# jeffersonfparil/poolgen

Measured on AMD Instinct MI355X. Metric: loci/sec ols_iter_with_kinship, 200 pools x 10M loci, higher is better.
Workload: dtype f64

## Files before the change

### poolgen_amd/csrc/pg_kinship.hip

```cpp
#include "pg_common.h"
#include <cstdlib>
#include <cstring>
#include <utility>

namespace {

#ifndef KIN_WAVES_DEF
#define KIN_WAVES_DEF 16
#endif
constexpr int KIN_WAVES = KIN_WAVES_DEF;
constexpr int KIN_THREADS = 64 * KIN_WAVES;
#ifndef KIN_RING_D
#define KIN_RING_D 3
#endif
constexpr int KIN_FUSE_MAXK = 2;
constexpr int KIN_TPW = 96 / KIN_WAVES;
#ifndef KIN_KC_DEF
#define KIN_KC_DEF 16
#endif
constexpr int KIN_KC = KIN_KC_DEF;
constexpr int KIN_PPT = (KIN_KC * 128 + KIN_THREADS - 1) / KIN_THREADS;

typedef double double4_t __attribute__((ext_vector_type(4)));
typedef unsigned int uint4_t __attribute__((ext_vector_type(4)));
typedef unsigned int uint2_t __attribute__((ext_vector_type(2)));

template <int CTRL, int ROW_MASK>
__device__ __forceinline__ double dpp_add(double v) {
    const int lo = __builtin_amdgcn_update_dpp(0, __double2loint(v), CTRL, ROW_MASK, 0xf, true);
    const int hi = __builtin_amdgcn_update_dpp(0, __double2hiint(v), CTRL, ROW_MASK, 0xf, true);
    return v + __hiloint2double(hi, lo);
}
template <int N>
__device__ __forceinline__ double row_from_plus(double v) {
    static_assert(N >= 1 && N <= 15, "row rotation");
    constexpr int CTRL = 0x120 + (16 - N);
    const int lo = __builtin_amdgcn_update_dpp(0, __double2loint(v), CTRL, 0xf, 0xf, false);
    const int hi = __builtin_amdgcn_update_dpp(0, __double2hiint(v), CTRL, 0xf, 0xf, false);
    return __hiloint2double(hi, lo);
}
template <int... I, typename F>
__device__ __forceinline__ void static_for_impl(std::integer_sequence<int, I...>, F &&f) {
    (f(std::integral_constant<int, I>{}), ...);
}
template <int N, typename F>
__device__ __forceinline__ void static_for(F &&f) {
    static_for_impl(std::make_integer_sequence<int, N>{}, f);
}
constexpr int kin_tri_ti(int t, int T) { int ti = 0; while (ti < T && t >= T - ti) { t -= T - ti; ++ti; } return ti < T ? ti : 0; }
constexpr int kin_tri_tj(int t, int T) { int ti = 0; while (ti < T && t >= T - ti) { t -= T - ti; ++ti; } return ti < T ? ti + t : 0; }
constexpr int kin_slot_tile(int w, int u, int T) { return (w + KIN_WAVES_DEF * u) < T * (T + 1) / 2 ? (w + KIN_WAVES_DEF * u) : 0; }

constexpr int KIN13_T[16][6][2] = {
    {{0, 0}, {0, 1}, {0, 2}, {1, 1}, {1, 2}, {2, 2}},
    {{3, 3}, {3, 4}, {3, 5}, {4, 4}, {4, 5}, {5, 5}},
    {{6, 6}, {6, 7}, {6, 8}, {7, 7}, {7, 8}, {8, 8}},
    {{9, 9}, {9, 10}, {9, 11}, {10, 10}, {10, 11}, {11, 11}},
    {{0, 3}, {0, 4}, {0, 5}, {1, 3}, {1, 4}, {1, 5}},
    {{0, 6}, {0, 7}, {0, 8}, {1, 6}, {1, 7}, {1, 8}},
    {{0, 9}, {0, 10}, {0, 11}, {1, 9}, {1, 10}, {1, 11}},
    {{3, 6}, {3, 7}, {3, 8}, {4, 6}, {4, 7}, {4, 8}},
    {{3, 9}, {3, 10}, {3, 11}, {4, 9}, {4, 10}, {4, 11}},
    {{6, 9}, {6, 10}, {6, 11}, {7, 9}, {7, 10}, {7, 11}},
    {{2, 4}, {2, 11}, {2, 12}, {4, 12}, {11, 12}, {12, 12}},
    {{2, 5}, {2, 6}, {2, 7}, {5, 6}, {5, 7}, {-1, -1}},
    {{0, 12}, {2, 3}, {3, 12}, {6, 12}, {7, 12}, {-1, -1}},
    {{5, 9}, {5, 10}, {5, 12}, {9, 12}, {10, 12}, {-1, -1}},
    {{2, 8}, {2, 9}, {2, 10}, {8, 9}, {8, 10}, {-1, -1}},
    {{1, 12}, {5, 8}, {5, 11}, {8, 11}, {8, 12}, {-1, -1}},
};
constexpr int kin13_ntiles(int w) { int c = 0; for (int u = 0; u < 6; ++u) c += KIN13_T[w][u][0] >= 0; return c; }
constexpr int kin13_col(int w, int idx) {
    int seen[12] = {-1, -1, -1, -1, -1, -1, -1, -1, -1, -1, -1, -1}, ns = 0;
    for (int u = 0; u < 6; ++u)
        for (int h = 0; h < 2; ++h) {
            const int c = KIN13_T[w][u][h];
            if (c < 0) continue;
            bool dup = false;
            for (int i = 0; i < ns; ++i) dup = dup || seen[i] == c;
            if (!dup) seen[ns++] = c;
        }
    return idx < ns ? seen[idx] : -1;
}
constexpr int kin13_ncols(int w) { int c = 0; while (c < 12 && kin13_col(w, c) >= 0) ++c; return c; }
constexpr int kin13_slot(int w, int col) { int i = 0; while (kin13_col(w, i) != col) ++i; return i; }
constexpr int KIN13_MAXC = 6;
constexpr int kin13_ndiag(int w) { int c = 0; for (int u = 0; u < 6; ++u) c += (KIN13_T[w][u][0] >= 0 && KIN13_T[w][u][0] == KIN13_T[w][u][1]); return c; }
constexpr int kin13_diag_index(int w, int u) { int c = 0; for (int v = 0; v < u; ++v) c += (KIN13_T[w][v][0] >= 0 && KIN13_T[w][v][0] == KIN13_T[w][v][1]); return c; }

struct KinParams {
    const double *G;
    int64_t p;
    int64_t ld;
    int64_t loci_per_wg;
    double *slabs;
    int n, T, npad, Tb, nb;
    int split;
    int merged;
    const double *ytil;
    double *spec;
    int k;
    int xcd_spx, npairs, nslab;
    int skip_dead;
    int wq_n[6], wq_first[6];
    int64_t wq_len[6];
};

template <bool FUSE, bool SPEC13, int SMALL = 0, bool SKIP = false, bool ODDN = true>
__global__ __launch_bounds__(KIN_THREADS, 1) void k_kinship_syrk(KinParams P) {
    extern __shared__ __attribute__((aligned(16))) double lds[];
    const int tid = threadIdx.x;
    const int lane = tid & 63;
    const int wave = tid >> 6;
    const int fi = lane & 15;
    const int kq = lane >> 4;

    int bx = blockIdx.x, by = blockIdx.y;
    if (P.xcd_spx) {
        const int xcd = blockIdx.x & 7, s = blockIdx.x >> 3, main = P.xcd_spx * P.npairs;
        if (s < main) { bx = xcd * P.xcd_spx + s / P.npairs; by = s % P.npairs; }
        else { const int e = (s - main) * 8 + xcd; bx = 8 * P.xcd_spx + e / P.npairs; by = e % P.npairs; }
        if (bx >= P.nslab) return;
    }
    int64_t loci_per_wg = P.loci_per_wg;
    if (P.wq_n[0] > 0) {
        int q = 0;
        while (q + 1 < P.npairs && (int)blockIdx.x >= P.wq_first[q + 1]) ++q;
        by = q;
        bx = (int)blockIdx.x - P.wq_first[q];
        loci_per_wg = P.wq_len[q];
    }
    int bi = 0, bj = 0;
    {
        int q = by / P.split;
        const int first = P.merged ? 1 : 0;
        for (bi = 0; bi < P.nb; ++bi) {
            const int cnt = P.nb - bi - first;
            if (q < cnt) { bj = bi + first + q; break; }
            q -= cnt;
        }
    }
    const bool diag = (bi == bj);
    const int Ta = min(P.Tb, P.T - bi * P.Tb);
    const int Tbb = min(P.Tb, P.T - bj * P.Tb);
    const int colsA = Ta * 16;
    const int colsB = diag ? 0 : Tbb * 16;
    int ldsld = colsA + colsB;
    if ((ldsld & 31) != 16) ldsld += 16;
    const int a0 = bi * P.Tb * 16;
    const int b0 = bj * P.Tb * 16;
    const int wa = min(colsA, P.n - a0);
    const int wb = diag ? 0 : min(colsB, P.n - b0);
    const int npa = (wa + 1) >> 1, npb = (wb + 1) >> 1;
    const int npr = npa + npb;

    const int nrect = diag ? 0 : Ta * Tbb;
    const int NA = Ta * (Ta + 1) / 2, NB = Tbb * (Tbb + 1) / 2, part = P.nb - 1;
    const int rankA = bj - 1, rankB = bi;
    const int cntA = P.merged ? (NA > rankA ? (NA - rankA + part - 1) / part : 0) : 0;
    const int cntB = P.merged ? (NB > rankB ? (NB - rankB + part - 1) / part : 0) : 0;
    const int ntiles = diag ? NA : nrect + cntA + cntB;
    const int split_id = by % P.split;
    int acol[KIN_TPW], bcol[KIN_TPW], orow[KIN_TPW], ocol[KIN_TPW];
    bool live[KIN_TPW];
#pragma unroll
    for (int u = 0; u < KIN_TPW; ++u) {
        const int t = split_id + P.split * (wave + KIN_WAVES * u);
        int ti = 0, tj = 0;
        live[u] = t < ntiles;
        int kind = diag ? 1 : 0;
        if (t < ntiles) {
            int q = t, Td = Ta;
            if (!diag && t >= nrect) {
                const bool inA = t - nrect < cntA;
                kind = inA ? 1 : 2;
                q = inA ? rankA + part * (t - nrect) : rankB + part * (t - nrect - cntA);
                Td = inA ? Ta : Tbb;
            }
            if (kind) {
                for (ti = 0; ti < Td; ++ti) {
                    const int cnt = Td - ti;
                    if (q < cnt) { tj = ti + q; break; }
                    q -= cnt;
                }
            } else {
                ti = t / Tbb;
                tj = t - ti * Tbb;
            }
        }
        acol[u] = (kind == 2 ? colsA : 0) + 16 * ti;
        bcol[u] = (kind == 1 ? 0 : colsA) + 16 * tj;
        orow[u] = (kind == 2 ? b0 : a0) + 16 * ti;
        ocol[u] = (kind == 1 ? a0 : b0) + 16 * tj;
    }

    int st_loc[KIN_PPT], st_lcol[KIN_PPT];
    int st_gcol[KIN_PPT];
    bool st_on[KIN_PPT], st_two[KIN_PPT];
#pragma unroll
    for (int r = 0; r < KIN_PPT; ++r) {
        const int t = tid + r * KIN_THREADS;
        const int loc = t / npr;
        const int q = t - loc * npr;
        st_on[r] = loc < KIN_KC;
        st_loc[r] = loc;
        int gcol, lcol;
        bool two;
        if (q < npa) {
            gcol = a0 + 2 * q; lcol = 2 * q; two = (2 * q + 1) < wa;
        } else {
            const int q2 = q - npa;
            gcol = b0 + 2 * q2; lcol = colsA + 2 * q2; two = (2 * q2 + 1) < wb;
        }
        st_lcol[r] = lcol;
        st_two[r] = two;
        st_gcol[r] = st_on[r] ? gcol : a0;
        if (!st_on[r]) st_loc[r] = 0;
    }

    const int64_t l_begin = (int64_t)bx * loci_per_wg;
    const int64_t l_end = min(P.p, l_begin + loci_per_wg);
    const int nstages = (l_end > l_begin) ? (int)((l_end - l_begin + KIN_KC - 1) / KIN_KC) : 0;
    const int bufsz = KIN_KC * ldsld;

    for (int i = tid; i < 2 * bufsz; i += KIN_THREADS) lds[i] = 0.0;
    double *ylds = lds + 2 * bufsz;
    if (FUSE)
        for (int i = tid; i < P.k * 256; i += KIN_THREADS) ylds[i] = P.ytil[i];
    __syncthreads();

    const uint64_t slab_bytes64 = (uint64_t)(l_end > l_begin ? l_end - l_begin : 0) * P.ld * 8;
    const __amdgpu_buffer_rsrc_t rsrc = __builtin_amdgcn_make_buffer_rsrc(
        const_cast<double *>(P.G + l_begin * P.ld), 0, (int)(uint32_t)slab_bytes64, 0x00020000);
    uint4_t stage_reg[KIN_PPT];
    uint32_t st_voff[KIN_PPT];
#pragma unroll
    for (int r = 0; r < KIN_PPT; ++r)
        st_voff[r] = st_on[r] ? (uint32_t)(((int64_t)st_loc[r] * P.ld + st_gcol[r]) * 8) : 0xFFFFFFF0u;
    const uint32_t stage_stride = (uint32_t)(KIN_KC * P.ld * 8);
    auto stage_load = [&](int c) {
#pragma unroll
        for (int r = 0; r < KIN_PPT; ++r)
            stage_reg[r] = __builtin_amdgcn_raw_buffer_load_b128(
                rsrc, st_on[r] ? st_voff[r] + (uint32_t)c * stage_stride : 0xFFFFFFF0u, 0, 0);
    };
    auto stage_store = [&](int buf) {
#pragma unroll
        for (int r = 0; r < KIN_PPT; ++r) {
            if (st_on[r]) {
                uint4_t v = stage_reg[r];
                if (!st_two[r]) { v.z = 0u; v.w = 0u; }
                *reinterpret_cast<uint4_t *>(&lds[buf * bufsz + st_loc[r] * ldsld + st_lcol[r]]) = v;
            }
        }
    };

    if (nstages > 0) {
        stage_load(0);
        stage_store(0);
    }
    __syncthreads();

    const int NV = 2 + P.k;
    double *scratch = ylds + KIN_FUSE_MAXK * 256 + wave * (4 * 64);
    double yreg[KIN_FUSE_MAXK][4];
#pragma unroll
    for (int t = 0; t < KIN_FUSE_MAXK; ++t)
#pragma unroll
        for (int j = 0; j < 4; ++j) yreg[t][j] = (FUSE && t < P.k) ? ylds[t * 256 + lane + 64 * j] : 0.0;
    auto spec_pass = [&](const double *buf, int64_t lbase) {
#pragma unroll
        for (int jl = 0; jl < KIN_KC / KIN_WAVES; ++jl) {
            const int loc = wave + KIN_WAVES * jl;
            const double *row = buf + loc * ldsld;
            const double shift = row[0];
            double s1 = 0.0, s2 = 0.0, sy[KIN_FUSE_MAXK], d[4];
#pragma unroll
            for (int t = 0; t < KIN_FUSE_MAXK; ++t) sy[t] = 0.0;
#pragma unroll
            for (int j = 0; j < 4; ++j) {
                const int pool = lane + 64 * j;
                if (SPEC13 && j < 3) d[j] = row[pool] - shift;
                else {
                    const double gv = row[pool < ldsld ? pool : ldsld - 1];
                    d[j] = (pool < P.n) ? gv - shift : 0.0;
                }
                s1 += d[j];
                s2 = fma(d[j], d[j], s2);
                sy[0] = fma(d[j], yreg[0][j], sy[0]);
            }
            const bool two = P.k > 1;
            if (two) {
#pragma unroll
                for (int j = 0; j < 4; ++j) sy[1] = fma(d[j], yreg[1][j], sy[1]);
            }
            scratch[lane] = s1;
            scratch[64 + lane] = s2;
            scratch[2 * 64 + lane] = sy[0];
            if (two) scratch[3 * 64 + lane] = sy[1];
            __builtin_amdgcn_wave_barrier();
            const int v = lane >> 4, r = lane & 15;
            const double *sc = scratch + v * 64 + r;
            double tot = (sc[0] + sc[16]) + (sc[32] + sc[48]);
            tot = dpp_add<0x111, 0xf>(tot);
            tot = dpp_add<0x112, 0xf>(tot);
            tot = dpp_add<0x114, 0xf>(tot);
            tot = dpp_add<0x118, 0xf>(tot);
            const int64_t l = lbase + loc;
            if (r == 15 && v < NV && l < l_end) P.spec[l * NV + v] = tot;
            __builtin_amdgcn_wave_barrier();
        }
    };

    auto run = [&](auto wc, auto tc) {
        constexpr int W = decltype(wc)::value;
        constexpr int TPW = decltype(tc)::value;
        constexpr int KS = KIN_KC / 4;
        constexpr int NQ = KS * TPW;
        constexpr int D = KIN_RING_D, R = KIN_RING_D + 1;
        static_assert(NQ % R == 0 && NQ > 2 * D, "ring indexing assumes the stage length is a multiple of the ring");
        double4_t acc[TPW];
#pragma unroll
        for (int u = 0; u < TPW; ++u) acc[u] = (double4_t){0.0, 0.0, 0.0, 0.0};
#ifndef KIN_SHARED_FRAGS
#define KIN_SHARED_FRAGS 1
#endif
        if constexpr (W >= 0 && KIN_SHARED_FRAGS) {
            constexpr int NC = kin13_ncols(W), NT = kin13_ntiles(W);
            static_assert(NC <= KIN13_MAXC && KS % 2 == 0, "fragment sets alternate with the k-step parity");
            constexpr int LD13 = 208, BUF13 = KIN_KC * LD13;
            auto ldv = [](const double *q) __attribute__((always_inline)) { return *(const volatile __attribute__((address_space(3))) double *)q; };
            double fr[2][KIN13_MAXC];
            const double *lb = lds + kq * LD13 + fi;
            constexpr bool has_strip = [] { bool h = false; for (int u = 0; u < 6; ++u) h = h || (KIN13_T[W][u][0] >= 0 && KIN13_T[W][u][0] < 12 && KIN13_T[W][u][1] == 12); return h; }();
            double bs[2][2];
            const double *lbs = lds + kq * LD13 + 192 + (lane & 3);
            constexpr int ND = (SMALL & 1) ? kin13_ndiag(W) : 0;
            double bd[2][ND > 0 ? ND : 1][2];
            const double *lbr1 = lds + kq * LD13 + ((fi + 4) & 15), *lbr2 = lds + kq * LD13 + ((fi + 8) & 15);
            auto load_set = [&](auto bc, auto sc, auto pc) __attribute__((always_inline)) {
                constexpr int s2 = decltype(sc)::value, par = decltype(pc)::value;
                constexpr int o = decltype(bc)::value * BUF13 + 4 * s2 * LD13;
                static_for<NC>([&](auto cc) __attribute__((always_inline)) {
                    constexpr int ci = decltype(cc)::value;
                    fr[par][ci] = ldv(lb + (o + 16 * kin13_col(W, ci)));
                });
                if constexpr ((SMALL & 2) != 0 && has_strip) {
                    bs[par][0] = ldv(lbs + o);
                    bs[par][1] = ldv(lbs + (o + 4));
                }
                if constexpr (ND > 0) {
                    static_for<NT>([&](auto uc) __attribute__((always_inline)) {
                        constexpr int u = decltype(uc)::value;
                        if constexpr (KIN13_T[W][u][0] == KIN13_T[W][u][1]) {
                            constexpr int di = kin13_diag_index(W, u);
                            bd[par][di][0] = ldv(lbr1 + (o + 16 * KIN13_T[W][u][0]));
                            bd[par][di][1] = ldv(lbr2 + (o + 16 * KIN13_T[W][u][0]));
                        }
                    });
                }
            };
            auto mfma_set = [&](auto pc) __attribute__((always_inline)) {
                constexpr int par = decltype(pc)::value;
                static_for<NT>([&](auto uc) __attribute__((always_inline)) {
                    constexpr int u = decltype(uc)::value;
                    constexpr int ti = KIN13_T[W][u][0], tj = KIN13_T[W][u][1];
                    const double fa = fr[par][kin13_slot(W, ti)];
                    if constexpr ((SMALL & 1) != 0 && ti == tj) {
                        acc[u][0] = __builtin_amdgcn_mfma_f64_4x4x4f64(fa, fa, acc[u][0], 0, 0, 0);
                        acc[u][1] = __builtin_amdgcn_mfma_f64_4x4x4f64(fa, bd[par][kin13_diag_index(W, u)][0], acc[u][1], 0, 0, 0);
                        acc[u][2] = __builtin_amdgcn_mfma_f64_4x4x4f64(fa, bd[par][kin13_diag_index(W, u)][1], acc[u][2], 0, 0, 0);
                    } else if constexpr ((SMALL & 2) != 0 && tj == 12 && ti != tj) {
                        acc[u][0] = __builtin_amdgcn_mfma_f64_4x4x4f64(fa, bs[par][0], acc[u][0], 0, 0, 0);
                        acc[u][1] = __builtin_amdgcn_mfma_f64_4x4x4f64(fa, bs[par][1], acc[u][1], 0, 0, 0);
                    } else {
                        acc[u] = __builtin_amdgcn_mfma_f64_16x16x4f64(fa, fr[par][kin13_slot(W, tj)], acc[u], 0, 0, 0);
                    }
                });
            };
            constexpr auto st_kind = [](int r) { const int t0 = W * 64 + r * KIN_THREADS; return t0 + 63 < KIN_KC * 97 ? 2 : (t0 >= KIN_KC * 104 ? 0 : 1); };
            uint4_t sreg[KIN_PPT];
            uint32_t voff[KIN_PPT];
            uint4_t *sdst[KIN_PPT];
#pragma unroll
            for (int r = 0; r < KIN_PPT; ++r) {
                sreg[r] = (uint4_t){0u, 0u, 0u, 0u};
                voff[r] = st_voff[r];
                sdst[r] = reinterpret_cast<uint4_t *>(&lds[st_loc[r] * LD13 + st_lcol[r]]);
            }
            auto st_load = [&]() __attribute__((always_inline)) {
                static_for<KIN_PPT>([&](auto rc) __attribute__((always_inline)) {
                    constexpr int r = decltype(rc)::value;
                    if constexpr (st_kind(r) == 2) {
                        voff[r] += stage_stride;
                        sreg[r] = __builtin_amdgcn_raw_buffer_load_b128(rsrc, voff[r], 0, 0);
                    } else if constexpr (st_kind(r) == 1) {
                        if (st_on[r]) {
                            voff[r] += stage_stride;
                            sreg[r] = __builtin_amdgcn_raw_buffer_load_b128(rsrc, voff[r], 0, 0);
                        }
                    }
                });
            };
            auto st_store = [&](auto bc) __attribute__((always_inline)) {
                constexpr int B = decltype(bc)::value;
                static_for<KIN_PPT>([&](auto rc) __attribute__((always_inline)) {
                    constexpr int r = decltype(rc)::value;
                    if constexpr (st_kind(r) != 0) {
                        uint4_t v = sreg[r];
                        if constexpr (ODDN) {
                            if (!st_two[r]) { v.z = 0u; v.w = 0u; }
                        }
                        if (st_kind(r) == 2 || st_on[r]) sdst[r][B * (BUF13 / 2)] = v;
                    }
                });
            };
            const double *srow = lds + lane, *srow3 = lds + (lane + 192 < P.n ? lane + 192 : 0);
            const bool sp_on = (lane & 15) == 15 && (lane >> 4) < NV;
            uint32_t sp_voff = (uint32_t)((W * NV + (lane >> 4)) * 8);
            const uint32_t sp_stride = (uint32_t)(KIN_KC * NV * 8);
            const __amdgpu_buffer_rsrc_t srsrc = __builtin_amdgcn_make_buffer_rsrc(
                FUSE ? P.spec + l_begin * NV : nullptr, 0, FUSE ? (int)(uint32_t)((uint64_t)(l_end > l_begin ? l_end - l_begin : 0) * NV * 8) : 0, 0x00020000);
            const double *sc13 = scratch + (lane >> 4) * 64 + (lane & 15);
            auto spec13 = [&](auto bc) __attribute__((always_inline)) {
                static_for<KIN_KC / KIN_WAVES>([&](auto jc) __attribute__((always_inline)) {
                    constexpr int jl = decltype(jc)::value;
                    constexpr int ro = decltype(bc)::value * BUF13 + (W + KIN_WAVES * jl) * LD13;
                    const double shift = ldv(lds + ro);
                    double s1 = 0.0, s2 = 0.0, sy[KIN_FUSE_MAXK], d[4];
#pragma unroll
                    for (int t = 0; t < KIN_FUSE_MAXK; ++t) sy[t] = 0.0;
#pragma unroll
                    for (int j = 0; j < 4; ++j) {
                        d[j] = (j < 3 ? ldv(srow + (ro + 64 * j)) : ldv(srow3 + ro)) - shift;
                        s1 += d[j];
                        s2 = fma(d[j], d[j], s2);
                        sy[0] = fma(d[j], yreg[0][j], sy[0]);
                    }
                    const bool two = P.k > 1;
                    if (two) {
#pragma unroll
                        for (int j = 0; j < 4; ++j) sy[1] = fma(d[j], yreg[1][j], sy[1]);
                    }
                    scratch[lane] = s1;
                    scratch[64 + lane] = s2;
                    scratch[2 * 64 + lane] = sy[0];
                    if (two) scratch[3 * 64 + lane] = sy[1];
                    __builtin_amdgcn_wave_barrier();
                    double tot = (sc13[0] + sc13[16]) + (sc13[32] + sc13[48]);
                    tot = dpp_add<0x111, 0xf>(tot);
                    tot = dpp_add<0x112, 0xf>(tot);
                    tot = dpp_add<0x114, 0xf>(tot);
                    tot = dpp_add<0x118, 0xf>(tot);
                    if (sp_on)
                        __builtin_amdgcn_raw_buffer_store_b64((uint2_t){(uint32_t)__double2loint(tot), (uint32_t)__double2hiint(tot)}, srsrc,
                                                              sp_voff + (uint32_t)(KIN_WAVES * jl * 8) * (uint32_t)NV, 0, 0);
                    __builtin_amdgcn_wave_barrier();
                });
                sp_voff += sp_stride;
            };
            constexpr int spec_step = (W / 4) % KS;
            auto stage = [&](auto bc, const auto more) __attribute__((always_inline)) {
                constexpr int B = decltype(bc)::value;
                if (more) st_load();
                static_for<KS>([&](auto sc) __attribute__((always_inline)) {
                    constexpr int s2 = decltype(sc)::value;
                    if constexpr (FUSE && s2 == spec_step) spec13(bc);
                    if constexpr (s2 + 1 < KS) {
                        load_set(bc, std::integral_constant<int, s2 + 1>{}, std::integral_constant<int, (s2 + 1) & 1>{});
                    } else {
                        if (more) st_store(std::integral_constant<int, B ^ 1>{});
                        __syncthreads();
                        if (more) load_set(std::integral_constant<int, B ^ 1>{}, std::integral_constant<int, 0>{}, std::integral_constant<int, 0>{});
                    }
                    mfma_set(std::integral_constant<int, s2 & 1>{});
                });
            };
            if (nstages > 0) load_set(std::integral_constant<int, 0>{}, std::integral_constant<int, 0>{}, std::integral_constant<int, 0>{});
            int c = 0;
            for (; c + 1 < nstages; c += 2) {
                stage(std::integral_constant<int, 0>{}, std::true_type{});
                stage(std::integral_constant<int, 1>{}, c + 2 < nstages);
            }
            if (c < nstages) stage(std::integral_constant<int, 0>{}, std::false_type{});
            double *slab = P.slabs + (size_t)bx * P.npad * P.npad;
            static_for<NT>([&](auto uc) __attribute__((always_inline)) {
                constexpr int u = decltype(uc)::value;
                constexpr int ti = KIN13_T[W][u][0], tj = KIN13_T[W][u][1];
                constexpr int r0 = 16 * ti, c0 = 16 * tj;
                const int bi = lane >> 4, bb = (lane >> 2) & 3, bj = lane & 3;
                if constexpr ((SMALL & 1) != 0 && ti == tj) {
                    slab[(size_t)(r0 + 4 * bb + bi) * P.npad + c0 + 4 * bb + bj] = acc[u][0];
                    if (bb < 3) slab[(size_t)(r0 + 4 * bb + bi) * P.npad + c0 + 4 * (bb + 1) + bj] = acc[u][1];
                    else slab[(size_t)(r0 + bj) * P.npad + c0 + 12 + bi] = acc[u][1];
                    if (bb < 2) slab[(size_t)(r0 + 4 * bb + bi) * P.npad + c0 + 4 * (bb + 2) + bj] = acc[u][2];
                } else if constexpr ((SMALL & 2) != 0 && tj == 12 && ti != tj) {
                    slab[(size_t)(r0 + 4 * bb + bi) * P.npad + c0 + bj] = acc[u][0];
                    slab[(size_t)(r0 + 4 * bb + bi) * P.npad + c0 + 4 + bj] = acc[u][1];
                } else {
#pragma unroll
                    for (int r = 0; r < 4; ++r) slab[(size_t)(r0 + kq + 4 * r) * P.npad + c0 + fi] = acc[u][r];
                }
            });
            return;
        }
        double fa[R], fb[R];
        const double *lanebase = lds + kq * ldsld + fi;
        auto frag_load = [&](const double *bufbase, auto qc) {
            constexpr int q = decltype(qc)::value;
            constexpr int s = q / TPW, u = q % TPW;
            if constexpr (W >= 0) {
                if constexpr (W + KIN_WAVES * u >= 91) return;
                constexpr int t = kin_slot_tile(W, u, 13);
                constexpr int ao = 4 * s * 208 + 16 * kin_tri_ti(t, 13);
                constexpr int bo = 4 * s * 208 + 16 * kin_tri_tj(t, 13);
                fa[q % R] = bufbase[ao];
                fb[q % R] = bufbase[bo];
            } else {
                if constexpr (SKIP) { if (!live[u]) return; }
                const double *row = bufbase + 4 * s * ldsld;
                fa[q % R] = row[acol[u]];
                fb[q % R] = row[bcol[u]];
            }
        };
        auto mfma_item = [&](auto qc) {
            constexpr int q = decltype(qc)::value;
            constexpr int u = q % TPW;
            if constexpr (W >= 0 && W + KIN_WAVES * u >= 91) return;
            if constexpr (W < 0 && SKIP) { if (!live[u]) return; }
            acc[u] = __builtin_amdgcn_mfma_f64_16x16x4f64(fa[q % R], fb[q % R], acc[u], 0, 0, 0);
        };
        if (nstages > 0)
            static_for<D>([&](auto qc) { frag_load(lanebase, qc); });
        for (int c = 0; c < nstages; ++c) {
            const bool more = (c + 1) < nstages;
            if (more) stage_load(c + 1);
            const double *buf = lds + (c & 1) * bufsz;
            const double *fb0 = lanebase + (c & 1) * bufsz;
            const double *fb1 = lanebase + ((c + 1) & 1) * bufsz;
#ifndef KIN_SPEC_STAGGER
#define KIN_SPEC_STAGGER 1
#endif
            constexpr int spec_at = (FUSE && W >= 0 && KIN_SPEC_STAGGER) ? ((W / 4) % 4) * ((NQ - D) / 4) : -1;
            static_for<NQ - D>([&](auto qc) {
                if constexpr (decltype(qc)::value == spec_at) spec_pass(buf, l_begin + (int64_t)c * KIN_KC);
                frag_load(fb0, std::integral_constant<int, decltype(qc)::value + D>{});
                mfma_item(qc);
            });
            if (more) stage_store((c + 1) & 1);
            if (FUSE && spec_at < 0) spec_pass(buf, l_begin + (int64_t)c * KIN_KC);
            __syncthreads();
            static_for<D>([&](auto dc) {
                constexpr int q = NQ - D + decltype(dc)::value;
                if (more) frag_load(fb1, std::integral_constant<int, q + D - NQ>{});
                mfma_item(std::integral_constant<int, q>{});
            });
        }
        double *slab = P.slabs + (size_t)bx * P.npad * P.npad;
        static_for<TPW>([&](auto uc) {
            constexpr int u = decltype(uc)::value;
            bool on;
            int r0, c0;
            if constexpr (W >= 0) {
                constexpr int t = W + KIN_WAVES * u;
                on = t < 91;
                r0 = 16 * kin_tri_ti(kin_slot_tile(W, u, 13), 13);
                c0 = 16 * kin_tri_tj(kin_slot_tile(W, u, 13), 13);
            } else {
                on = live[u]; r0 = orow[u]; c0 = ocol[u];
            }
            if (on) {
#pragma unroll
                for (int r = 0; r < 4; ++r) slab[(size_t)(r0 + kq + 4 * r) * P.npad + c0 + fi] = acc[u][r];
            }
        });
    };
    if constexpr (SPEC13) {
        switch (wave) {
        case 0: run(std::integral_constant<int, 0>{}, std::integral_constant<int, KIN_TPW>{}); break;
        case 1: run(std::integral_constant<int, 1>{}, std::integral_constant<int, KIN_TPW>{}); break;
        case 2: run(std::integral_constant<int, 2>{}, std::integral_constant<int, KIN_TPW>{}); break;
        case 3: run(std::integral_constant<int, 3>{}, std::integral_constant<int, KIN_TPW>{}); break;
        case 4: run(std::integral_constant<int, 4>{}, std::integral_constant<int, KIN_TPW>{}); break;
        case 5: run(std::integral_constant<int, 5>{}, std::integral_constant<int, KIN_TPW>{}); break;
        case 6: run(std::integral_constant<int, 6>{}, std::integral_constant<int, KIN_TPW>{}); break;
#if KIN_WAVES_DEF == 8
        default: run(std::integral_constant<int, 7>{}, std::integral_constant<int, KIN_TPW>{}); break;
#else
        case 7: run(std::integral_constant<int, 7>{}, std::integral_constant<int, KIN_TPW>{}); break;
        case 8: run(std::integral_constant<int, 8>{}, std::integral_constant<int, KIN_TPW>{}); break;
        case 9: run(std::integral_constant<int, 9>{}, std::integral_constant<int, KIN_TPW>{}); break;
        case 10: run(std::integral_constant<int, 10>{}, std::integral_constant<int, KIN_TPW>{}); break;
        case 11: run(std::integral_constant<int, 11>{}, std::integral_constant<int, KIN_TPW>{}); break;
        case 12: run(std::integral_constant<int, 12>{}, std::integral_constant<int, KIN_TPW>{}); break;
        case 13: run(std::integral_constant<int, 13>{}, std::integral_constant<int, KIN_TPW>{}); break;
        case 14: run(std::integral_constant<int, 14>{}, std::integral_constant<int, KIN_TPW>{}); break;
        default: run(std::integral_constant<int, 15>{}, std::integral_constant<int, KIN_TPW>{}); break;
#endif
        }
    } else {
        constexpr std::integral_constant<int, -1> any{};
        switch ((ntiles + KIN_WAVES - 1) / KIN_WAVES) {
        case 0: case 1: case 2: run(any, std::integral_constant<int, 2>{}); break;
        case 3: run(any, std::integral_constant<int, 3>{}); break;
        case 4: run(any, std::integral_constant<int, 4>{}); break;
        case 5: run(any, std::integral_constant<int, 5>{}); break;
        default: run(any, std::integral_constant<int, KIN_TPW>{}); break;
        }
    }
}

constexpr double KIN_PAIR_FLOOR = 2.7;
struct KinCounts { int blk, nb, n[6]; };
__global__ __launch_bounds__(256) void k_kinship_reduce(const double *__restrict__ slabs, int nslabs, int npad, int n,
                                                        double add_const, double *__restrict__ S, const KinCounts C) {
    __shared__ double part[4][64];
    const int jj = threadIdx.x & 63, grp = threadIdx.x >> 6;
    const int j = blockIdx.x * 64 + jj;
    const int i = blockIdx.y;
    const bool on = i < n && j < n && i <= j;
    double s = 0.0;
    if (on && C.blk) {
        const int bi = i / C.blk, bj = j / C.blk;
        nslabs = C.n[bi * C.nb - bi * (bi - 1) / 2 + (bj - bi)];
    }
    if (on) {
        const size_t off = (size_t)i * npad + j;
        const size_t stride = (size_t)npad * npad;
        for (int w = grp; w < nslabs; w += 4) s += slabs[w * stride + off];
    }
    part[grp][jj] = s;
    __syncthreads();
    if (on && grp == 0) {
        const double t = ((part[0][jj] + part[1][jj]) + (part[2][jj] + part[3][jj])) + add_const;
        S[(size_t)i * n + j] = t;
        S[(size_t)j * n + i] = t;
    }
}

}

#ifndef KIN_LAUNCH_NAME
#define KIN_LAUNCH_NAME pg_launch_kinship
#endif
int KIN_LAUNCH_NAME(pg_ctx *ctx, const double *G, int64_t p, int n, int64_t ld, double *S,
                      bool add_intercept, int kid, bool allow_fuse) {
#if KIN_WAVES_DEF == 16
    if (n <= 64) return pg_launch_kinship_w8(ctx, G, p, n, ld, S, add_intercept, kid, allow_fuse);
#endif

    PG_CHECK(ctx, G && S, "kinship: null pointer");
    PG_CHECK(ctx, p > 0 && n > 0, "kinship: need p > 0 and n > 0 (p=%lld n=%d)", (long long)p, n);
    PG_CHECK(ctx, ld >= n && (ld % 2) == 0, "kinship: ld (%lld) must be even and >= n (%d)",
             (long long)ld, n);
    PG_CHECK(ctx, (reinterpret_cast<uintptr_t>(G) & 15) == 0, "kinship: G must be 16-byte aligned");
    PG_HIP(ctx, hipSetDevice(ctx->device));
    const int cus = ctx->cus;

    KinParams P;
    P.G = G; P.p = p; P.ld = ld; P.n = n;
    P.T = (n + 15) / 16;
    P.npad = P.T * 16;
    if (P.T <= 13) { P.Tb = P.T; P.nb = 1; }
    else { P.Tb = 8; P.nb = (P.T + 7) / 8; }
    P.merged = (P.nb >= 4 || (P.nb == 2 && P.T >= 15)) ? 1 : 0;
    if (!P.merged && P.nb >= 2 && P.nb <= 3) {
        double best = 1e30;
        int best_tb = P.Tb;
        for (int tb = (P.T + P.nb - 1) / P.nb; tb <= 8; ++tb) {
            double units = 0.0;
            for (int bi = 0; bi < P.nb; ++bi)
                for (int bj = bi; bj < P.nb; ++bj) {
                    const int Ta = std::min(tb, P.T - bi * tb), Tbb = std::min(tb, P.T - bj * tb);
                    if (Ta <= 0 || Tbb <= 0) { units += 1e6; continue; }
                    const int tiles = bi == bj ? Ta * (Ta + 1) / 2 : Ta * Tbb;
                    units += std::max(KIN_PAIR_FLOOR, (double)((tiles + KIN_WAVES - 1) / KIN_WAVES));
                }
            if (units <= best) { best = units; best_tb = tb; }
        }
        P.Tb = best_tb;
    }
    P.split = (P.merged && P.nb == 2) ? 2 : 1;
    const int npairs = (P.merged ? P.nb * (P.nb - 1) / 2 : P.nb * (P.nb + 1) / 2) * P.split;
    int nslab = cus / npairs;
    if (nslab < 1) nslab = 1;
    const int64_t max_slabs = (p + KIN_KC - 1) / KIN_KC;
    if (nslab > max_slabs) nslab = (int)max_slabs;
    P.loci_per_wg = (p + nslab - 1) / nslab;
    P.loci_per_wg = (P.loci_per_wg + KIN_KC - 1) / KIN_KC * KIN_KC;
    const int64_t max_loci_per_wg = ((int64_t)0xFFFFFFF0 / (ld * 8)) / KIN_KC * KIN_KC - KIN_KC;
    if (P.loci_per_wg > max_loci_per_wg) P.loci_per_wg = max_loci_per_wg;
    nslab = (int)((p + P.loci_per_wg - 1) / P.loci_per_wg);

    P.npairs = npairs; P.nslab = nslab;
    P.skip_dead = P.nb <= 2 ? 1 : 0;
    P.xcd_spx = 0;
    if (npairs > 1 && cus % 8 == 0) {
        const int spx = (cus / 8) / npairs;
        if (spx >= 1 && 8 * spx <= nslab) P.xcd_spx = spx;
    }
    for (int q = 0; q < 6; ++q) { P.wq_n[q] = 0; P.wq_first[q] = 0; P.wq_len[q] = 0; }
    KinCounts KC;
    KC.blk = 0; KC.nb = P.nb;
    for (int q = 0; q < 6; ++q) KC.n[q] = 0;
    int grid1d = 0;
    if (P.nb >= 2 && P.nb <= 3 && !P.merged) {
        double wgt[6], wsum = 0.0;
        int q = 0;
        for (int bi = 0; bi < P.nb; ++bi)
            for (int bj = bi; bj < P.nb; ++bj, ++q) {
                const int Ta = std::min(P.Tb, P.T - bi * P.Tb), Tbb = std::min(P.Tb, P.T - bj * P.Tb);
                const int tiles = bi == bj ? Ta * (Ta + 1) / 2 : Ta * Tbb;
                wgt[q] = std::max(KIN_PAIR_FLOOR, (double)((tiles + KIN_WAVES - 1) / KIN_WAVES)) + 0.35;
                wsum += wgt[q];
            }
        int used = 0;
        for (q = 0; q < npairs; ++q) { P.wq_n[q] = std::max(1, (int)(cus * wgt[q] / wsum)); used += P.wq_n[q]; }
        for (int left = cus - used; left > 0; --left) {
            int best = 0;
            for (q = 1; q < npairs; ++q)
                if (wgt[q] / P.wq_n[q] > wgt[best] / P.wq_n[best]) best = q;
            ++P.wq_n[best];
        }
        int first = 0, maxn = 0;
        for (q = 0; q < npairs; ++q) {
            int64_t len = (p + P.wq_n[q] - 1) / P.wq_n[q];
            len = (len + KIN_KC - 1) / KIN_KC * KIN_KC;
            if (len > max_loci_per_wg) len = max_loci_per_wg;
            P.wq_len[q] = len;
            P.wq_n[q] = (int)((p + len - 1) / len);
            P.wq_first[q] = first;
            first += P.wq_n[q];
            maxn = std::max(maxn, P.wq_n[q]);
            KC.n[q] = P.wq_n[q];
        }
        grid1d = first;
        nslab = maxn;
        P.nslab = nslab;
        P.xcd_spx = 0;
        P.skip_dead = 0;
        KC.blk = P.Tb * 16;
    }
    const size_t slab_bytes = (size_t)nslab * P.npad * P.npad * sizeof(double);
    int rc = pg_ws_reserve(ctx, slab_bytes);
    if (rc) return rc;
    P.slabs = static_cast<double *>(ctx->ws.get());

    int ldsld = (P.nb == 1) ? P.Tb * 16 : 2 * P.Tb * 16;
    if ((ldsld & 31) != 16) ldsld += 16;
    const size_t fuse_lds = (size_t)2 * KIN_KC * ldsld * 8 + ((size_t)KIN_FUSE_MAXK * 256 + (size_t)KIN_WAVES * 4 * 64) * 8;
    const bool fuse = allow_fuse && ctx->ph_armed && fuse_lds <= 160 * 1024 && P.nb == 1 && ctx->ph_n == n && ctx->ph_k >= 1 && ctx->ph_k <= KIN_FUSE_MAXK &&
                      ctx->ph_ytil_dev != nullptr;
    P.ytil = nullptr; P.spec = nullptr; P.k = 0;
    ctx->spec_valid = false;
    if (fuse) {
        const size_t need = (size_t)p * (2 + ctx->ph_k) * sizeof(double);
        const int rrc = ctx->spec_dev.reserve(ctx, need, "kinship");
        if (rrc) return rrc;
        P.ytil = ctx->ph_ytil_dev; P.spec = ctx->spec_dev; P.k = ctx->ph_k;
    }
    const size_t shmem = (size_t)2 * KIN_KC * ldsld * sizeof(double) + (fuse ? ((size_t)KIN_FUSE_MAXK * 256 + (size_t)KIN_WAVES * 4 * 64) * sizeof(double) : 0);
    const int max_cols = (P.nb == 1) ? P.Tb * 16 : 2 * P.Tb * 16;
    PG_CHECK(ctx, KIN_KC * (max_cols / 2) <= KIN_PPT * KIN_THREADS, "kinship: staging overflow");
    const bool spec13 = (P.nb == 1 && P.T == 13);
    auto launch = [&](auto kern) -> hipError_t {
        hipError_t e = hipFuncSetAttribute(reinterpret_cast<const void *>(kern),
                                           hipFuncAttributeMaxDynamicSharedMemorySize, (int)shmem);
        if (e != hipSuccess) return e;
        if (grid1d) hipLaunchKernelGGL(kern, dim3(grid1d), dim3(KIN_THREADS), shmem, ctx->stream, P);
        else if (P.xcd_spx) hipLaunchKernelGGL(kern, dim3(8 * ((P.xcd_spx * npairs) + ((nslab - 8 * P.xcd_spx) * npairs + 7) / 8)), dim3(KIN_THREADS), shmem,
                                          ctx->stream, P);
        else hipLaunchKernelGGL(kern, dim3(nslab, npairs), dim3(KIN_THREADS), shmem, ctx->stream, P);
        return hipSuccess;
    };
    pg_prof_begin(ctx, kid);
    hipError_t le;
    auto pick = [&](auto fz) -> hipError_t {
        constexpr bool FZ = decltype(fz)::value;
        if (!spec13) return P.skip_dead ? launch(k_kinship_syrk<FZ, false, 0, true>) : launch(k_kinship_syrk<FZ, false, 0, false>);
        if (n & 1) return n <= 200 ? launch(k_kinship_syrk<FZ, true, 3>) : launch(k_kinship_syrk<FZ, true, 1>);
        return n <= 200 ? launch(k_kinship_syrk<FZ, true, 3, false, false>) : launch(k_kinship_syrk<FZ, true, 1, false, false>);
    };
    le = fuse ? pick(std::true_type{}) : pick(std::false_type{});
    PG_HIP(ctx, le);
    pg_prof_end(ctx);
    PG_HIP(ctx, hipGetLastError());
    if (fuse) {
        ctx->spec_G = G; ctx->spec_p = p; ctx->spec_ld = ld; ctx->spec_n = n; ctx->spec_k = ctx->ph_k;
        ctx->spec_valid = true;
    }
    pg_prof_begin(ctx, PG_K_KINSHIP_REDUCE);
    hipLaunchKernelGGL(k_kinship_reduce, dim3((n + 63) / 64, n), dim3(256), 0, ctx->stream,
                       P.slabs, nslab, P.npad, n, add_intercept ? 1.0 : 0.0, S, KC);
    pg_prof_end(ctx);
    PG_HIP(ctx, hipGetLastError());
    return PG_OK;
}

#ifndef KIN_NO_EXPORTS
extern "C" int pg_kinship_partial_dev(pg_ctx *ctx, const double *G_dev, int64_t p, int n,
                                      int64_t ld, double *S_dev) {
    if (!ctx) return PG_ERR_INVALID;
    return pg_launch_kinship(ctx, G_dev, p, n, ld, S_dev, false, PG_K_KINSHIP, true);
}

extern "C" int pg_gp_xxt_dev(pg_ctx *ctx, const double *G_dev, int64_t p, int n, int64_t ld,
                             double *XXt_dev) {
    if (!ctx) return PG_ERR_INVALID;
    return pg_launch_kinship(ctx, G_dev, p, n, ld, XXt_dev, true, PG_K_GP_XXT);
}

extern "C" int pg_set_phenotypes(pg_ctx *ctx, int n, const double *Y, int k) {
    if (!ctx) return PG_ERR_INVALID;
    const int rc = pg_phenotypes_upload(ctx, n, Y, k);
    ctx->ph_armed = rc == PG_OK && ctx->ph_n > 0;
    return rc;
}

int pg_phenotypes_upload(pg_ctx *ctx, int n, const double *Y, int k) {
    ctx->spec_valid = false;
    if (n > 0 && Y && ctx->ph_n == n && ctx->ph_k == k && ctx->ph_ytil_dev && ctx->ph_Y.size() == (size_t)n * k &&
        std::memcmp(ctx->ph_Y.data(), Y, sizeof(double) * n * k) == 0)
        return PG_OK;
    if (ctx->ph_n > 0) ++ctx->ph_serial;
    ctx->ph_n = 0; ctx->ph_k = 0; ctx->ph_Y.clear();
    if (n == 0 || !Y) return PG_OK;
    PG_CHECK(ctx, n >= 2 && k >= 1, "set_phenotypes: bad shape n=%d k=%d", n, k);
    if (k > 4 || n > 256) return PG_OK;
    for (int i = 0; i < n * k; ++i)
        PG_CHECK(ctx, Y[i] == Y[i], "set_phenotypes: phenotype matrix contains NaN; remove pools with "
                                    "missing phenotypes first (gwas/ols.rs:287)");
    PG_HIP(ctx, hipSetDevice(ctx->device));
    std::vector<double> yt((size_t)k * 256, 0.0);
    for (int t = 0; t < k; ++t) {
        double mu = 0.0;
        for (int i = 0; i < n; ++i) mu += Y[(size_t)i * k + t];
        mu /= n;
        double syy = 0.0;
        for (int i = 0; i < n; ++i) {
            const double y = Y[(size_t)i * k + t] - mu;
            yt[(size_t)t * 256 + i] = y;
            syy += y * y;
        }
        ctx->ph_syy[t] = syy;
    }
    const int rc = ctx->ph_ytil_dev.reserve(ctx, sizeof(double) * 4 * 256, "set_phenotypes");
    if (rc) return rc;
    PG_HIP(ctx, hipMemcpyAsync(ctx->ph_ytil_dev, yt.data(), sizeof(double) * k * 256, hipMemcpyHostToDevice, ctx->stream));
    PG_HIP(ctx, hipStreamSynchronize(ctx->stream));
    ctx->ph_Y.assign(Y, Y + (size_t)n * k);
    ctx->ph_n = n; ctx->ph_k = k;
    return PG_OK;
}
#endif
```

Before: 1.362 billion.

## Split fused spec13 reductions into reads/sums and interleave with MFMA halves

The fused per-locus spec reduction is split into an LDS-read phase and a sums phase. Each is placed between two halves of the MFMA set at staggered k-step slots per wave group, so LDS latency and DPP reductions overlap with matrix work instead of stalling one k-step. The global store of the totals is deferred to the start of the next stage. It also adds optional s_memtime stamp instrumentation behind a macro, at the cost of extra register pressure for the held values.

```diff
diff --git a/poolgen_amd/csrc/pg_kinship.hip b/poolgen_amd/csrc/pg_kinship.hip
--- a/poolgen_amd/csrc/pg_kinship.hip
+++ b/poolgen_amd/csrc/pg_kinship.hip
@@ -104,7 +104,23 @@
     int skip_dead;
     int wq_n[6], wq_first[6];
     int64_t wq_len[6];
+#ifdef KIN_STAMP
+    unsigned long long *stamps;
+#endif
 };
+
+#ifdef KIN_STAMP
+constexpr int KIN_NSTAMP = 8;
+#define KIN_TS(i)                                                         \
+    do {                                                                  \
+        __builtin_amdgcn_sched_barrier(0);                                \
+        const unsigned long long ts_now_ = __builtin_amdgcn_s_memtime();  \
+        ts[i] = ts_on ? ts_now_ : ts[i];                                  \
+        __builtin_amdgcn_sched_barrier(0);                                \
+    } while (0)
+#else
+#define KIN_TS(i) do { } while (0)
+#endif
 
 template <bool FUSE, bool SPEC13, int SMALL = 0, bool SKIP = false, bool ODDN = true>
 __global__ __launch_bounds__(KIN_THREADS, 1) void k_kinship_syrk(KinParams P) {
@@ -360,10 +376,11 @@
                     });
                 }
             };
-            auto mfma_set = [&](auto pc) __attribute__((always_inline)) {
-                constexpr int par = decltype(pc)::value;
-                static_for<NT>([&](auto uc) __attribute__((always_inline)) {
-                    constexpr int u = decltype(uc)::value;
+            constexpr int NTH = NT / 2;
+            auto mfma_half = [&](auto pc, auto hc) __attribute__((always_inline)) {
+                constexpr int par = decltype(pc)::value, u0 = decltype(hc)::value ? NTH : 0;
+                static_for<(decltype(hc)::value ? NT - NTH : NTH)>([&](auto uc) __attribute__((always_inline)) {
+                    constexpr int u = u0 + decltype(uc)::value;
                     constexpr int ti = KIN13_T[W][u][0], tj = KIN13_T[W][u][1];
                     const double fa = fr[par][kin13_slot(W, ti)];
                     if constexpr ((SMALL & 1) != 0 && ti == tj) {
@@ -422,17 +439,53 @@
             const __amdgpu_buffer_rsrc_t srsrc = __builtin_amdgcn_make_buffer_rsrc(
                 FUSE ? P.spec + l_begin * NV : nullptr, 0, FUSE ? (int)(uint32_t)((uint64_t)(l_end > l_begin ? l_end - l_begin : 0) * NV * 8) : 0, 0x00020000);
             const double *sc13 = scratch + (lane >> 4) * 64 + (lane & 15);
-            auto spec13 = [&](auto bc) __attribute__((always_inline)) {
-                static_for<KIN_KC / KIN_WAVES>([&](auto jc) __attribute__((always_inline)) {
+#ifndef KIN_SUMS_DEFER
+#define KIN_SUMS_DEFER 1
+#endif
+            constexpr int NJL = KIN_KC / KIN_WAVES;
+#ifdef KIN_STAMP
+            unsigned long long ts[KIN_NSTAMP] = {0, 0, 0, 0, 0, 0, 0, 0};
+            bool ts_on = false;
+#endif
+            double sp_tot[NJL], sp_g[NJL][5];
+#pragma unroll
+            for (int jl = 0; jl < NJL; ++jl) sp_tot[jl] = 0.0;
+            if constexpr (KIN_SUMS_DEFER) sp_voff -= sp_stride;
+            auto spec_store = [&]() __attribute__((always_inline)) {
+                static_for<NJL>([&](auto jc) __attribute__((always_inline)) {
+                    constexpr int jl = decltype(jc)::value;
+                    if (sp_on)
+                        __builtin_amdgcn_raw_buffer_store_b64((uint2_t){(uint32_t)__double2loint(sp_tot[jl]), (uint32_t)__double2hiint(sp_tot[jl])},
+                                                              srsrc, sp_voff + (uint32_t)(KIN_WAVES * jl * 8) * (uint32_t)NV, 0, 0);
+                });
+                KIN_TS(3);
+                sp_voff += sp_stride;
+            };
+            auto spec_reads = [&](auto bc) __attribute__((always_inline)) {
+                KIN_TS(0);
+                static_for<NJL>([&](auto jc) __attribute__((always_inline)) {
                     constexpr int jl = decltype(jc)::value;
                     constexpr int ro = decltype(bc)::value * BUF13 + (W + KIN_WAVES * jl) * LD13;
-                    const double shift = ldv(lds + ro);
+                    sp_g[jl][4] = ldv(lds + ro);
+#pragma unroll
+                    for (int j = 0; j < 4; ++j) sp_g[jl][j] = j < 3 ? ldv(srow + (ro + 64 * j)) : ldv(srow3 + ro);
+                });
+                __builtin_amdgcn_sched_barrier(0);
+            };
+            auto spec_sums = [&]() __attribute__((always_inline)) {
+#ifdef KIN_STAMP
+                asm volatile("s_waitcnt lgkmcnt(0)" ::: "memory");
+                KIN_TS(1);
+#endif
+                static_for<NJL>([&](auto jc) __attribute__((always_inline)) {
+                    constexpr int jl = decltype(jc)::value;
+                    const double shift = sp_g[jl][4];
                     double s1 = 0.0, s2 = 0.0, sy[KIN_FUSE_MAXK], d[4];
 #pragma unroll
                     for (int t = 0; t < KIN_FUSE_MAXK; ++t) sy[t] = 0.0;
 #pragma unroll
                     for (int j = 0; j < 4; ++j) {
-                        d[j] = (j < 3 ? ldv(srow + (ro + 64 * j)) : ldv(srow3 + ro)) - shift;
+                        d[j] = sp_g[jl][j] - shift;
                         s1 += d[j];
                         s2 = fma(d[j], d[j], s2);
                         sy[0] = fma(d[j], yreg[0][j], sy[0]);
@@ -448,41 +501,73 @@
                     if (two) scratch[3 * 64 + lane] = sy[1];
                     __builtin_amdgcn_wave_barrier();
                     double tot = (sc13[0] + sc13[16]) + (sc13[32] + sc13[48]);
+                    KIN_TS(2);
                     tot = dpp_add<0x111, 0xf>(tot);
                     tot = dpp_add<0x112, 0xf>(tot);
                     tot = dpp_add<0x114, 0xf>(tot);
                     tot = dpp_add<0x118, 0xf>(tot);
-                    if (sp_on)
-                        __builtin_amdgcn_raw_buffer_store_b64((uint2_t){(uint32_t)__double2loint(tot), (uint32_t)__double2hiint(tot)}, srsrc,
-                                                              sp_voff + (uint32_t)(KIN_WAVES * jl * 8) * (uint32_t)NV, 0, 0);
+                    sp_tot[jl] = tot;
                     __builtin_amdgcn_wave_barrier();
                 });
-                sp_voff += sp_stride;
+                if constexpr (!KIN_SUMS_DEFER) spec_store();
+                __builtin_amdgcn_sched_barrier(0);
             };
-            constexpr int spec_step = (W / 4) % KS;
+#ifndef KIN_SUMS_EARLY
+#define KIN_SUMS_EARLY 1
+#endif
+            constexpr int sp_grp = (W / 4) % 4;
+#ifndef KIN_SUMS_SLOTS
+#define KIN_SUMS_SLOTS {0, 2, 4, 3}
+#endif
+            constexpr int sp_slots[4] = KIN_SUMS_SLOTS;
+            constexpr int sums_at = KIN_SUMS_EARLY ? sp_slots[sp_grp] : 2 * (sp_grp % KS);
+            constexpr int reads_at = (KIN_SUMS_EARLY && sp_grp != 0 && sums_at > 0) ? sums_at - 1 : sums_at;
+            static_assert(!KIN_SUMS_EARLY || (KS >= 4 && sums_at <= 2 * (KS - 2)), "the sums end in front of the last k-step's fragment reads");
             auto stage = [&](auto bc, const auto more) __attribute__((always_inline)) {
                 constexpr int B = decltype(bc)::value;
+                if constexpr (FUSE && KIN_SUMS_DEFER) spec_store();
                 if (more) st_load();
                 static_for<KS>([&](auto sc) __attribute__((always_inline)) {
                     constexpr int s2 = decltype(sc)::value;
-                    if constexpr (FUSE && s2 == spec_step) spec13(bc);
+                    if constexpr (FUSE && 2 * s2 == reads_at) spec_reads(bc);
+                    if constexpr (FUSE && 2 * s2 == sums_at) spec_sums();
                     if constexpr (s2 + 1 < KS) {
                         load_set(bc, std::integral_constant<int, s2 + 1>{}, std::integral_constant<int, (s2 + 1) & 1>{});
                     } else {
+                        KIN_TS(4);
                         if (more) st_store(std::integral_constant<int, B ^ 1>{});
+                        KIN_TS(5);
+                        KIN_TS(6);
                         __syncthreads();
+                        KIN_TS(7);
                         if (more) load_set(std::integral_constant<int, B ^ 1>{}, std::integral_constant<int, 0>{}, std::integral_constant<int, 0>{});
                     }
-                    mfma_set(std::integral_constant<int, s2 & 1>{});
+                    mfma_half(std::integral_constant<int, s2 & 1>{}, std::integral_constant<int, 0>{});
+                    if constexpr (FUSE && 2 * s2 + 1 == reads_at) spec_reads(bc);
+                    if constexpr (FUSE && 2 * s2 + 1 == sums_at) spec_sums();
+                    mfma_half(std::integral_constant<int, s2 & 1>{}, std::integral_constant<int, 1>{});
                 });
             };
             if (nstages > 0) load_set(std::integral_constant<int, 0>{}, std::integral_constant<int, 0>{}, std::integral_constant<int, 0>{});
             int c = 0;
             for (; c + 1 < nstages; c += 2) {
+#ifdef KIN_STAMP
+                ts_on = c == (nstages / 2 & ~1);
+#endif
                 stage(std::integral_constant<int, 0>{}, std::true_type{});
+#ifdef KIN_STAMP
+                ts_on = false;
+#endif
                 stage(std::integral_constant<int, 1>{}, c + 2 < nstages);
             }
             if (c < nstages) stage(std::integral_constant<int, 0>{}, std::false_type{});
+            if constexpr (FUSE && KIN_SUMS_DEFER) spec_store();
+#ifdef KIN_STAMP
+            if (FUSE && P.stamps && lane == 0) {
+#pragma unroll
+                for (int i = 0; i < KIN_NSTAMP; ++i) P.stamps[((size_t)bx * KIN_WAVES + W) * KIN_NSTAMP + i] = ts[i];
+            }
+#endif
             double *slab = P.slabs + (size_t)bx * P.npad * P.npad;
             static_for<NT>([&](auto uc) __attribute__((always_inline)) {
                 constexpr int u = decltype(uc)::value;
@@ -638,7 +723,21 @@
     }
 }
 
-}
+#ifdef KIN_STAMP
+unsigned long long *g_kin_stamps = nullptr;
+size_t g_kin_stamps_cap = 0, g_kin_stamps_n = 0;
+#endif
+
+}
+
+#if defined(KIN_STAMP) && !defined(KIN_NO_EXPORTS)
+extern "C" long pg_kin_stamps_read(unsigned long long *out, long cap) {
+    if (!g_kin_stamps || hipDeviceSynchronize() != hipSuccess) return -1;
+    const long n = std::min<long>(cap, (long)g_kin_stamps_n);
+    if (hipMemcpy(out, g_kin_stamps, (size_t)n * sizeof(unsigned long long), hipMemcpyDeviceToHost) != hipSuccess) return -1;
+    return n;
+}
+#endif
 
 #ifndef KIN_LAUNCH_NAME
 #define KIN_LAUNCH_NAME pg_launch_kinship
@@ -752,6 +851,9 @@
     const bool fuse = allow_fuse && ctx->ph_armed && fuse_lds <= 160 * 1024 && P.nb == 1 && ctx->ph_n == n && ctx->ph_k >= 1 && ctx->ph_k <= KIN_FUSE_MAXK &&
                       ctx->ph_ytil_dev != nullptr;
     P.ytil = nullptr; P.spec = nullptr; P.k = 0;
+#ifdef KIN_STAMP
+    P.stamps = nullptr;
+#endif
     ctx->spec_valid = false;
     if (fuse) {
         const size_t need = (size_t)p * (2 + ctx->ph_k) * sizeof(double);
@@ -763,7 +865,21 @@
     const int max_cols = (P.nb == 1) ? P.Tb * 16 : 2 * P.Tb * 16;
     PG_CHECK(ctx, KIN_KC * (max_cols / 2) <= KIN_PPT * KIN_THREADS, "kinship: staging overflow");
     const bool spec13 = (P.nb == 1 && P.T == 13);
-    auto launch = [&](auto kern) -> hipError_t {
+#ifdef KIN_STAMP
+    if (fuse && spec13) {
+        const size_t need = (size_t)nslab * KIN_WAVES * KIN_NSTAMP;
+        if (need > g_kin_stamps_cap) {
+            if (g_kin_stamps) PG_HIP(ctx, hipFree(g_kin_stamps));
+            g_kin_stamps = nullptr; g_kin_stamps_cap = 0;
+            PG_HIP(ctx, hipMalloc(&g_kin_stamps, need * sizeof(unsigned long long)));
+            g_kin_stamps_cap = need;
+        }
+        g_kin_stamps_n = need;
+        PG_HIP(ctx, hipMemsetAsync(g_kin_stamps, 0, need * sizeof(unsigned long long), ctx->stream));
+        P.stamps = g_kin_stamps;
+    }
+#endif
+    auto launch =[&](auto kern) -> hipError_t {
         hipError_t e = hipFuncSetAttribute(reinterpret_cast<const void *>(kern),
                                            hipFuncAttributeMaxDynamicSharedMemorySize, (int)shmem);
         if (e != hipSuccess) return e;
```

New measurement: 1.328 billion. -2.5%, worse.
